# google/libultrahdr

Measured on AMD Instinct MI355X. Metric: Mpixels/s encode+decode (API-1 P010+YUV420, 4K), device-resident round trip, higher is better.
Workload: dtype f32; 1 GPU; API-1 3840x2160 round trip per step: encode (P010 HLG + YCbCr420 -> two-pass 3-ch gain map at scale 1, FDCT q95, Huffman: two JPEG scans) + decode (Huffman, IDCT, applyGainMap -> RGBA_F16 linear); frames resident in HBM

## Files before the change

### libultrahdr_amd/csrc/api_entropy.cpp

```cpp
#include "api_internal.h"

#include <condition_variable>
#include <functional>
#include <mutex>

uhdr_error_info_t uhdr_api::check_scan(const uhdr_hip_jpeg_scan_t* sc, bool need_coef, int* mcus_per_row, int* mcu_rows, int* blocks_per_mcu) {
  if (!sc) return err_status(UHDR_CODEC_INVALID_PARAM, "received nullptr for the scan description");
  if (sc->num_components != 1 && sc->num_components != 3)
    return err_status(UHDR_CODEC_INVALID_PARAM, "a scan has 1 or 3 components, received %d", sc->num_components);
  if (sc->w == 0 || sc->h == 0 || sc->w > 65535 || sc->h > 65535)
    return err_status(UHDR_CODEC_INVALID_PARAM, "image dimensions %ux%u are outside JPEG's 1..65535", sc->w, sc->h);
  int hmax = 1, vmax = 1, bpm = 0;
  for (int i = 0; i < sc->num_components; i++) {
    const int hs = sc->num_components == 1 ? 1 : sc->h_samp[i], vs = sc->num_components == 1 ? 1 : sc->v_samp[i];
    if (hs < 1 || hs > 2 || vs < 1 || vs > 2) return err_status(UHDR_CODEC_INVALID_PARAM, "component %d: sampling factors %dx%d not in {1, 2}", i, hs, vs);
    if (hs > hmax) hmax = hs;
    if (vs > vmax) vmax = vs;
    bpm += hs * vs;
    if (need_coef && (!sc->coef[i] || ((uintptr_t)sc->coef[i] & 15)))
      return err_status(UHDR_CODEC_INVALID_PARAM, "coefficient buffer %d is null or not 16-byte aligned", i);
    if (sc->blocks_w[i] < 1 || sc->blocks_h[i] < 1) return err_status(UHDR_CODEC_INVALID_PARAM, "component %d: empty block grid", i);
  }
  if (sc->num_components == 1) {
    *mcus_per_row = sc->blocks_w[0];
    *mcu_rows = sc->blocks_h[0];
    if ((unsigned)sc->blocks_w[0] != (sc->w + 7) / 8 || (unsigned)sc->blocks_h[0] != (sc->h + 7) / 8)
      return err_status(UHDR_CODEC_INVALID_PARAM, "a %dx%d block grid does not match a %ux%u image", sc->blocks_w[0], sc->blocks_h[0], sc->w, sc->h);
  } else {
    *mcus_per_row = (int)((sc->w + 8u * hmax - 1) / (8u * hmax));
    *mcu_rows = (int)((sc->h + 8u * vmax - 1) / (8u * vmax));
    for (int i = 0; i < 3; i++) {
      const unsigned cw = (sc->w * sc->h_samp[i] + hmax - 1) / hmax, chh = (sc->h * sc->v_samp[i] + vmax - 1) / vmax;
      const int min_w = (int)((cw + 7) / 8), min_h = (int)((chh + 7) / 8);
      if (sc->blocks_w[i] < min_w || sc->blocks_w[i] > *mcus_per_row * sc->h_samp[i] || sc->blocks_h[i] < min_h ||
          sc->blocks_h[i] > *mcu_rows * sc->v_samp[i])
        return err_status(UHDR_CODEC_INVALID_PARAM, "component %d: a %dx%d block grid does not match a %ux%u image at %dx%d sampling", i,
                          sc->blocks_w[i], sc->blocks_h[i], sc->w, sc->h, sc->h_samp[i], sc->v_samp[i]);
    }
  }
  *blocks_per_mcu = bpm;
  return ok_status();
}

static hipError_t wait_stream(uhdr_hip_ctx* c) {
  static const int spin_us = [] { const char* e = getenv("UHDR_HIP_SYNC_SPIN_US"); return e ? atoi(e) : 2000; }();
  if (spin_us > 0) {
    const auto t0 = std::chrono::steady_clock::now();
    for (;;) {
      const hipError_t q = hipStreamQuery(c->stream);
      if (q == hipSuccess) return hipSuccess;
      if (q != hipErrorNotReady) return q;
      if (std::chrono::steady_clock::now() - t0 > std::chrono::microseconds(spin_us)) break;
    }
  }
  return hipStreamSynchronize(c->stream);
}


uhdr_error_info_t uhdr_hip_huffman_encode_dev(uhdr_hip_ctx_t* c, const uhdr_hip_jpeg_scan_t* sc, uint8_t* out, size_t out_capacity,
                                              size_t* out_bytes) {
  if (!c) return err_status(UHDR_CODEC_INVALID_PARAM, "received nullptr for uhdr_hip context");
  if (!out || !out_bytes) return err_status(UHDR_CODEC_INVALID_PARAM, "received nullptr for the output buffer or size");
  int mpr = 0, mrows = 0, bpm = 0;
  UHDR_TRY(check_scan(sc, true, &mpr, &mrows, &bpm));
  const bool stream = sc->restart_interval == 0;
  if (!stream && (sc->restart_interval < 1 || sc->restart_interval > 65535 || sc->restart_interval * bpm > 64))
    return err_status(UHDR_CODEC_UNSUPPORTED_FEATURE, "restart_interval must be 0 (no markers) or in 1..%d for %d blocks per MCU (one wavefront "
                      "encodes one restart interval of at most 64 blocks); received %d", 64 / bpm, bpm, sc->restart_interval);
  if (stream && 2 * bpm > 64) return err_status(UHDR_CODEC_UNSUPPORTED_FEATURE, "%d blocks per MCU: outside the HIP path", bpm);
  HIP_TRY(hipSetDevice(c->device));
  if (!c->d_huff) {
    std::vector<uint32_t> blob(host::jpeg_huff_code_tables());
    blob.resize((size_t)host::kHuffTabWords + 16);
    memcpy(blob.data() + host::kHuffTabWords, host::jpeg_zigzag_to_natural(), 64);
    HIP_TRY(hipMalloc((void**)&c->d_huff, blob.size() * sizeof(uint32_t)));
    HIP_TRY(hipMemcpyAsync(c->d_huff, blob.data(), blob.size() * sizeof(uint32_t), hipMemcpyHostToDevice, c->stream));
    HIP_TRY(hipStreamSynchronize(c->stream));
  }
  HuffArgs a;
  memset(&a, 0, sizeof a);
  a.ncomp = sc->num_components;
  for (int i = 0; i < a.ncomp; i++) {
    a.coef[i] = sc->coef[i];
    a.bw[i] = sc->blocks_w[i]; a.bh[i] = sc->blocks_h[i];
    a.hs[i] = a.ncomp == 1 ? 1 : sc->h_samp[i]; a.vs[i] = a.ncomp == 1 ? 1 : sc->v_samp[i];
  }
  a.mcus_per_row = mpr;
  a.total_mcus = mpr * mrows;
  a.ri = stream ? huff_stream_segment_mcus(bpm) : sc->restart_interval;
  a.blocks_per_mcu = bpm;
  a.nseg = (a.total_mcus + a.ri - 1) / a.ri;
  a.tables = c->d_huff;
  a.zigzag = (const uint8_t*)(c->d_huff + host::kHuffTabWords);
  if (stream) {
    if (out_capacity > 0xFFFFFFF0u) out_capacity = 0xFFFFFFF0u;
    HuffStream t;
    memset(&t, 0, sizeof t);
    t.raw_words = ((uint64_t)out_capacity + 3) / 4 + 1;
    const uint64_t worst_words = (uint64_t)a.total_mcus * bpm * 52 + 2;
    if (t.raw_words > worst_words) t.raw_words = worst_words;
    const int nchunks = huff_stuff_chunks(t.raw_words * 4u);
    UHDR_TRY(ensure(c->scratch[4], (size_t)t.raw_words * 4));
    UHDR_TRY(ensure(c->scratch[5], ((size_t)a.nseg + 2) * sizeof(uint64_t) + (4 + (size_t)a.nseg + (size_t)nchunks) * sizeof(uint32_t)));
    t.raw = (uint32_t*)c->scratch[4].p;
    t.seg_start = (uint64_t*)c->scratch[5].p;
    uint64_t* d_total = t.seg_start + (size_t)a.nseg + 1;
    t.meta = (uint32_t*)(d_total + 1);
    t.seg_bits = t.meta + 4;
    uint32_t* chunk_counts = t.seg_bits + a.nseg;
    if (!c->huff_two_pass) {
      const size_t need = huff_stream_slot_bytes(a.nseg);
      if (c->huff_slots.cap >= need || !c->huff_slots_refused || need < c->huff_slots_refused) {
        if (ensure(c->huff_slots, need).error_code == UHDR_CODEC_OK) {
          t.slots = (uint32_t*)c->huff_slots.p;
        } else {
          (void)hipGetLastError();
          c->huff_slots_refused = need;
          fprintf(stderr, "uhdr_hip: no device memory for %zu bytes of Huffman segment slots: marker-less scans of that size take the two-pass route\n", need);
        }
      }
    }
    if (c->huff_route_log) fprintf(stderr, "uhdr_hip: huffman_encode stream route=%s nseg=%d\n", t.slots ? "one_walk" : "two_pass", a.nseg);
    {
      ProfScope ps(c, "huffman_encode");
      HIP_TRY(launch_huffman_encode_stream(a, t, chunk_counts, d_total, out, (uint64_t)out_capacity, c->stream));
    }
    c->stats.entropy_encode_stream++;
    if (!c->h_flags) HIP_TRY(hipHostMalloc((void**)&c->h_flags, 64 * sizeof(uint32_t), hipHostMallocDefault));
    uint32_t* hp = c->h_flags + 48;
    HIP_TRY(hipMemcpyAsync(hp, d_total, sizeof(uint64_t) + 4 * sizeof(uint32_t), hipMemcpyDeviceToHost, c->stream));
    HIP_TRY(wait_stream(c));
    uint64_t total = 0;
    uint32_t meta[4] = {0, 0, 0, 0};
    memcpy(&total, hp, sizeof total);
    memcpy(meta, hp + 2, sizeof meta);
    if (meta[2]) return err_status(UHDR_CODEC_INVALID_PARAM, "coefficients outside the baseline range (DC difference beyond 11 bits / AC beyond 10 bits)");
    const uint64_t raw_bytes = ((((uint64_t)meta[1] << 32) | meta[0]) + 7) / 8;
    if (raw_bytes > t.raw_words * 4u) total = raw_bytes + raw_bytes / 64 + 64;
    *out_bytes = (size_t)total;
    if (total > out_capacity)
      return err_status(UHDR_CODEC_MEM_ERROR, "entropy-coded data needs %llu bytes, the output buffer holds %zu", (unsigned long long)total, out_capacity);
    return ok_status();
  }
  a.slot_stride = huff_slot_stride();
  UHDR_TRY(ensure(c->scratch[4], (size_t)a.nseg * a.slot_stride));
  const size_t meta = (size_t)a.nseg * sizeof(uint32_t) + 16 + ((size_t)a.nseg + 1) * sizeof(uint64_t) + 16;
  UHDR_TRY(ensure(c->scratch[5], meta));
  a.slots = (uint8_t*)c->scratch[4].p;
  uint64_t* offsets = (uint64_t*)c->scratch[5].p;
  uint32_t* status = (uint32_t*)(offsets + (size_t)a.nseg + 1);
  a.seg_bytes = status + 2;
  {
    ProfScope ps(c, "huffman_encode");
    HIP_TRY(launch_huffman_encode(a, offsets, status, out, (uint64_t)out_capacity, c->stream));
  }
  c->stats.entropy_encode_intervals++;
  uint64_t total = 0;
  uint32_t bad = 0;
  HIP_TRY(hipMemcpyAsync(&total, offsets + a.nseg, sizeof total, hipMemcpyDeviceToHost, c->stream));
  HIP_TRY(hipMemcpyAsync(&bad, status, sizeof bad, hipMemcpyDeviceToHost, c->stream));
  HIP_TRY(wait_stream(c));
  if (bad) return err_status(UHDR_CODEC_INVALID_PARAM, "coefficients outside the baseline range (DC difference beyond 11 bits / AC beyond 10 bits)");
  *out_bytes = (size_t)total;
  if (total > out_capacity)
    return err_status(UHDR_CODEC_MEM_ERROR, "entropy-coded data needs %llu bytes, the output buffer holds %zu", (unsigned long long)total, out_capacity);
  return ok_status();
}

static bool make_dec_table(const uint8_t bits[17], const uint8_t vals[256], HuffDecTable* t) {
  memset(t, 0, sizeof *t);
  int nsym = 0;
  for (int l = 1; l <= 16; l++) nsym += bits[l];
  if (nsym > 256) return false;
  int code = 0, k = 0;
  for (int l = 1; l <= 16; l++) {
    if (bits[l]) {
// ... 744 lines not shown
```

### libultrahdr_amd/csrc/huffman_encode.hip

```cpp
#include "lds_copy.h"
#include "wg_scan.h"
#include "uhdr_types.h"

namespace uhdr {
namespace {

constexpr int kSegBlocks = 64;
constexpr int kWordsPerBlock = 52;
constexpr int kCoefRow = 33;

__device__ __forceinline__ uint32_t wave_incl_scan(uint32_t v, uint32_t lane) {
#pragma unroll
  for (int d = 1; d < 64; d <<= 1) {
    const uint32_t y = (uint32_t)__shfl_up((int)v, d, 64);
    if (lane >= (uint32_t)d) v += y;
  }
  return v;
}

__device__ __forceinline__ uint64_t zigzag_nonzero_map(const uint32_t* s_coef, uint32_t zz_of_lane, uint32_t lane) {
  uint64_t mine = 0;
  const uint32_t word = zz_of_lane >> 1, sh = (zz_of_lane & 1u) * 16u;
#pragma unroll 4
  for (uint32_t b = 0; b < (uint32_t)kSegBlocks; b++) {
    const uint32_t v = (s_coef[b * kCoefRow + word] >> sh) & 0xffffu;
    const uint64_t m = __builtin_amdgcn_ballot_w64(v != 0);
    if (lane == b) mine = m;
  }
  return mine;
}
template <typename Put>
__device__ __forceinline__ void walk_block(const uint32_t* dct, const uint32_t* act, int dc_diff, bool real, const uint32_t* coef_row,
                                           const uint8_t* zz, uint64_t nz, uint32_t& out_of_range, Put put) {
  int temp = dc_diff, temp2 = dc_diff;
  if (temp < 0) { temp = -temp; temp2--; }
  uint32_t nbits = 32u - (uint32_t)__clz(temp);
  out_of_range |= nbits > 11u;
  uint32_t e = dct[nbits & 15u];
  put(e & 0xffffu, e >> 16);
  if (nbits) put((uint32_t)temp2 & ((1u << nbits) - 1u), nbits);
  uint32_t prev = 0;
  if (real) {
    uint64_t m = nz & ~1ull;
    while (m != 0) {
      const uint32_t k = (uint32_t)__builtin_ctzll(m);
      m &= m - 1ull;
      uint32_t r = k - prev - 1u;
      prev = k;
      const uint32_t idx = zz[k];
      const uint32_t wd = coef_row[idx >> 1];
      temp = (idx & 1u) ? ((int)wd >> 16) : (int)(int16_t)(wd & 0xffffu);
      while (r > 15) {
        e = act[0xf0];
        put(e & 0xffffu, e >> 16);
        r -= 16;
      }
      temp2 = temp;
      if (temp < 0) { temp = -temp; temp2--; }
      nbits = 32u - (uint32_t)__clz(temp);
      out_of_range |= nbits > 10u;
      e = act[((r << 4) + nbits) & 255u];
      put(e & 0xffffu, e >> 16);
      put((uint32_t)temp2 & ((1u << (nbits & 31u)) - 1u), nbits);
    }
  }
  if (prev < 63u) {
    e = act[0];
    put(e & 0xffffu, e >> 16);
  }
}

constexpr int kWordsSmall = 16;
constexpr uint32_t kRetry = 0xFFFFFFFEu, kBadCoef = 0xFFFFFFFFu;

template <int WORDS, bool RETRY>
__global__ __launch_bounds__(64) void huff_encode_kernel(const HuffArgs a) {
  __shared__ __attribute__((aligned(16))) uint32_t s_tab[2 * (16 + 256)];
  __shared__ uint32_t s_coef[kSegBlocks * kCoefRow];
  __shared__ uint32_t s_bits[kSegBlocks * WORDS + 2];
  __shared__ int s_dc[kSegBlocks];
  __shared__ int s_real[kSegBlocks];
  __shared__ uint32_t s_gbits[kSegBlocks];
  __shared__ uint8_t s_zz[64];
  const uint32_t lane = threadIdx.x;
  copy_words_to_lds<4>(s_tab, a.tables, 2 * (16 + 256), lane, 64);
  s_zz[lane] = a.zigzag[lane];
  const int bpm = a.blocks_per_mcu;
  const int per = a.ri * bpm;
  const int G = (RETRY || per > 32) ? 1 : 64 / per;
  const uint32_t group_words = (uint32_t)(kSegBlocks * WORDS) / (uint32_t)G;
  const int nwseg = (a.nseg + G - 1) / G;

  for (int wseg = (int)blockIdx.x; wseg < nwseg; wseg += (int)gridDim.x) {
    __syncthreads();
    const int g = (int)lane / per, l = (int)lane - g * per;
    const int seg = wseg * G + g;
    if constexpr (RETRY) {
      if (a.seg_bytes[wseg] != kRetry) continue;
    }
    const int mcu_local = l / bpm, k_in_mcu = l - mcu_local * bpm;
    const int mcu = seg * a.ri + mcu_local;
    const bool active = g < G && seg < a.nseg && mcu_local < a.ri && mcu < a.total_mcus;
    int c = 0, kk = k_in_mcu;
    if (a.ncomp > 1) {
      while (c < a.ncomp - 1 && kk >= a.hs[c] * a.vs[c]) { kk -= a.hs[c] * a.vs[c]; c++; }
    }
    const int hs = a.ncomp > 1 ? a.hs[c] : 1, vs = a.ncomp > 1 ? a.vs[c] : 1;
    const int yi = kk / hs, xi = kk - yi * hs;
    const int my = mcu / a.mcus_per_row, mx = mcu - my * a.mcus_per_row;
    const int by = my * vs + yi, bx = mx * hs + xi;
    const bool real = active && by < a.bh[c] && bx < a.bw[c];
    uint32_t* crow = s_coef + lane * kCoefRow;
    if (real) {
      const uint4* src = (const uint4*)(a.coef[c] + ((size_t)by * a.bw[c] + bx) * 64);
#pragma unroll
      for (int i = 0; i < 8; i++) {
        const uint4 q = src[i];
        crow[4 * i] = q.x; crow[4 * i + 1] = q.y; crow[4 * i + 2] = q.z; crow[4 * i + 3] = q.w;
      }
    }
    s_real[lane] = real ? 1 : 0;
    s_dc[lane] = real ? (int)(int16_t)(crow[0] & 0xffffu) : 0;
    __syncthreads();
    int dcv = s_dc[lane];
    if (active && !real) {
      for (int d = 1; d <= 3; d++) {
        if (k_in_mcu >= d && s_real[lane - d]) { dcv = s_dc[lane - d]; break; }
      }
    }
    __syncthreads();
    s_dc[lane] = dcv;
    __syncthreads();
    int pred = 0;
    if (active) {
      if (kk > 0) pred = s_dc[lane - 1];
      else if (mcu_local > 0) pred = s_dc[(int)lane - bpm + hs * vs - 1];
    }
    const uint32_t* dct = s_tab + (c ? (16 + 256) : 0);
    const uint32_t* act = dct + 16;
    const int diff = dcv - pred;
    const uint64_t nz = zigzag_nonzero_map(s_coef, s_zz[lane], lane);

    uint32_t len = 0, oob = 0;
    if (active) walk_block(dct, act, diff, real, crow, s_zz, nz, oob, [&](uint32_t, uint32_t n) { len += n; });
    const uint32_t incl = wave_incl_scan(len, lane);
    const int first = g * per, last = min(first + per - 1, 63);
    const uint32_t v_before = (uint32_t)__shfl((int)incl, min(max(first - 1, 0), 63), 64);
    const uint32_t v_last = (uint32_t)__shfl((int)incl, last, 64);
    const uint32_t before = (first > 0 && first < 64) ? v_before : 0u;
    const uint32_t total_bits = g < G ? v_last - before : 0u;
    const uint32_t off = incl - len - before;
    const uint32_t cap_bits = group_words * 32u;
    if (__builtin_amdgcn_ballot_w64(oob != 0) != 0) {
      if (l == 0 && g < G && seg < a.nseg) a.seg_bytes[seg] = kBadCoef;
      continue;
    }
    const bool fits = total_bits <= cap_bits;
    if (l == 0 && g < G) s_gbits[g] = fits ? total_bits : 0xFFFFFFFFu;
    for (uint32_t i = lane; i < (uint32_t)(kSegBlocks * WORDS) + 2u; i += 64) s_bits[i] = 0u;
    __syncthreads();

    const uint32_t gbase = (uint32_t)g * group_words;
    if (active && fits) {
      uint64_t acc = 0;
      uint32_t cnt = off & 31u, w = gbase + (off >> 5);
      walk_block(dct, act, diff, real, crow, s_zz, nz, oob, [&](uint32_t code, uint32_t n) {
        acc = (acc << n) | (uint64_t)code;
        cnt += n;
        if (cnt >= 32u) {
          cnt -= 32u;
          atomicOr(&s_bits[w++], (uint32_t)(acc >> cnt));
        }
      });
      if (cnt) atomicOr(&s_bits[w], (uint32_t)(acc << (32u - cnt)));
    }
    __syncthreads();
    if (l == 0 && g < G && fits && (total_bits & 7u)) {
      const uint32_t pad = 8u - (total_bits & 7u), pos = total_bits & 31u;
      atomicOr(&s_bits[gbase + (total_bits >> 5)], ((1u << pad) - 1u) << (32u - pos - pad));
    }
    __syncthreads();

    for (int gg = 0; gg < G; gg++) {
      const int sg = wseg * G + gg;
      if (sg >= a.nseg) break;
      const uint32_t tb = s_gbits[gg];
      if (tb == 0xFFFFFFFFu) {
        if (lane == 0) a.seg_bytes[sg] = RETRY ? kBadCoef : kRetry;
        continue;
      }
      const uint32_t nbytes = (tb + 7u) >> 3;
      const uint32_t* bits = s_bits + (uint32_t)gg * group_words;
      uint8_t* dst = a.slots + (size_t)sg * a.slot_stride;
      uint32_t carry = 0;
      for (uint32_t base = 0; base < nbytes; base += 256) {
        const uint32_t i0 = base + lane * 4;
        const uint32_t wd = i0 < nbytes ? bits[i0 >> 2] : 0u;
        const uint32_t nv = i0 < nbytes ? min(nbytes - i0, 4u) : 0u;
        uint32_t b[4], nff = 0;
#pragma unroll
        for (int k = 0; k < 4; k++) {
          b[k] = (wd >> (24 - 8 * k)) & 0xffu;
          if ((uint32_t)k < nv && b[k] == 0xffu) nff++;
        }
        const uint32_t incl_ff = wave_incl_scan(nff, lane);
        uint32_t pos = i0 + carry + (incl_ff - nff);
#pragma unroll
        for (int k = 0; k < 4; k++) {
          if ((uint32_t)k < nv) {
            dst[pos++] = (uint8_t)b[k];
            if (b[k] == 0xffu) dst[pos++] = 0;
          }
        }
        carry += (uint32_t)__shfl((int)incl_ff, 63, 64);
      }
      if (lane == 0) a.seg_bytes[sg] = nbytes + carry;
    }
  }
}

__global__ __launch_bounds__(1024) void huff_offsets_kernel(const uint32_t* __restrict__ seg_bytes, int nseg, uint64_t* __restrict__ offsets,
                                                            uint32_t* __restrict__ status) {
  __shared__ uint64_t s_sum[1024];
  __shared__ uint32_t s_bad;
  const int tid = (int)threadIdx.x;
  if (tid == 0) s_bad = 0;
  __syncthreads();
  const int per = (nseg + 1023) / 1024, lo = min(tid * per, nseg), hi = min(lo + per, nseg);
  uint64_t sum = 0;
  bool bad = false;
  for (int i = lo; i < hi; i++) {
    const uint32_t n = seg_bytes[i];
    bad |= n >= kRetry;
    sum += (uint64_t)n + 2u;
  }
  if (bad) atomicOr(&s_bad, 1u);
  s_sum[tid] = sum;
  __syncthreads();
  for (int d = 1; d < 1024; d <<= 1) {
    const uint64_t y = tid >= d ? s_sum[tid - d] : 0;
    __syncthreads();
    s_sum[tid] += y;
    __syncthreads();
  }
  uint64_t run = s_sum[tid] - sum;
  for (int i = lo; i < hi; i++) {
    offsets[i] = run;
    run += (uint64_t)seg_bytes[i] + 2u;
  }
  if (tid == 1023) offsets[nseg] = s_sum[1023] - 2u;
  if (tid == 0) *status = s_bad;
}

__global__ __launch_bounds__(256) void huff_gather_kernel(const uint8_t* __restrict__ slots, uint32_t slot_stride,
                                                          const uint32_t* __restrict__ seg_bytes, const uint64_t* __restrict__ offsets, int nseg,
                                                          uint8_t* __restrict__ out, uint64_t cap) {
  for (int seg = (int)blockIdx.x; seg < nseg; seg += (int)gridDim.x) {
    const uint32_t n = seg_bytes[seg];
    const uint64_t off = offsets[seg];
    if (n >= kRetry || off + n + 2u > cap + (seg == nseg - 1 ? 2u : 0u)) continue;
    const uint8_t* src = slots + (size_t)seg * slot_stride;
    for (uint32_t i = threadIdx.x; i < n; i += 256) out[off + i] = src[i];
    if (threadIdx.x == 0 && seg < nseg - 1) {
      out[off + n] = 0xff;
      out[off + n + 1] = (uint8_t)(0xd0 + (seg & 7));
    }
  }
}


constexpr int kStuffChunk = 4096;

template <int WORDS, int PASS>
__global__ __launch_bounds__(64) void huff_stream_kernel(const HuffArgs a, const HuffStream t) {
  __shared__ __attribute__((aligned(16))) uint32_t s_tab[2 * (16 + 256)];
  __shared__ uint32_t s_coef[kSegBlocks * kCoefRow];
  __shared__ uint32_t s_bits[PASS == 0 ? 1 : kSegBlocks * WORDS + 2];
  __shared__ int s_dc[kSegBlocks];
  __shared__ int s_real[kSegBlocks];
  __shared__ uint8_t s_zz[64];
  const uint32_t lane = threadIdx.x;
  if constexpr (PASS == 2) {
    if (t.meta[3] == 0) return;
  }
  copy_words_to_lds<4>(s_tab, a.tables, 2 * (16 + 256), lane, 64);
  s_zz[lane] = a.zigzag[lane];
  const int bpm = a.blocks_per_mcu;
  constexpr uint32_t kCapBits = (uint32_t)(kSegBlocks * WORDS) * 32u;
  for (int seg = (int)blockIdx.x; seg < a.nseg; seg += (int)gridDim.x) {
    __syncthreads();
    uint64_t start = 0;
    uint32_t seg_total = 0;
    if constexpr (PASS != 0) {
      seg_total = t.seg_bits[seg];
      start = t.seg_start[seg];
      const bool small = seg_total + 32u <= (uint32_t)(kSegBlocks * kWordsSmall) * 32u;
      if (seg_total >= kRetry || small != (PASS == 1)) continue;
    }
    const int mcu_local = (int)lane / bpm, k_in_mcu = (int)lane - mcu_local * bpm;
    const int mcu = seg * a.ri + mcu_local - 1;
    const bool valid = mcu_local <= a.ri && mcu >= 0 && mcu < a.total_mcus;
    const bool emits = valid && mcu_local >= 1;
    int c = 0, kk = k_in_mcu;
    if (a.ncomp > 1) {
      while (c < a.ncomp - 1 && kk >= a.hs[c] * a.vs[c]) { kk -= a.hs[c] * a.vs[c]; c++; }
    }
    const int hs = a.ncomp > 1 ? a.hs[c] : 1, vs = a.ncomp > 1 ? a.vs[c] : 1;
    const int yi = kk / hs, xi = kk - yi * hs;
    const int mcu_c = valid ? mcu : 0;
    const int my = mcu_c / a.mcus_per_row, mx = mcu_c - my * a.mcus_per_row;
    const int by = my * vs + yi, bx = mx * hs + xi;
    const bool real = valid && by < a.bh[c] && bx < a.bw[c];
    uint32_t* crow = s_coef + lane * kCoefRow;
    if (real) {
      const uint4* src = (const uint4*)(a.coef[c] + ((size_t)by * a.bw[c] + bx) * 64);
      if (emits) {
#pragma unroll
        for (int i = 0; i < 8; i++) {
          const uint4 q = src[i];
          crow[4 * i] = q.x; crow[4 * i + 1] = q.y; crow[4 * i + 2] = q.z; crow[4 * i + 3] = q.w;
        }
      } else {
        crow[0] = *(const uint32_t*)src;
      }
    }
    s_real[lane] = real ? 1 : 0;
    s_dc[lane] = real ? (int)(int16_t)(crow[0] & 0xffffu) : 0;
    __syncthreads();
    int dcv = s_dc[lane];
    if (valid && !real) {
      for (int d = 1; d <= 3; d++) {
        if (k_in_mcu >= d && s_real[lane - d]) { dcv = s_dc[lane - d]; break; }
      }
    }
    __syncthreads();
    s_dc[lane] = dcv;
    __syncthreads();
    int pred = 0;
    if (emits) {
      if (kk > 0) pred = s_dc[lane - 1];
      else pred = s_dc[(int)lane - bpm + hs * vs - 1];
    }
    const uint32_t* dct = s_tab + (c ? (16 + 256) : 0);
    const uint32_t* act = dct + 16;
    const int diff = dcv - pred;
    const uint64_t nz = zigzag_nonzero_map(s_coef, s_zz[lane], lane);
    uint32_t len = 0, oob = 0;
    if (emits) walk_block(dct, act, diff, real, crow, s_zz, nz, oob, [&](uint32_t, uint32_t n) { len += n; });
    const uint32_t incl = wave_incl_scan(len, lane);
    const uint32_t total_bits = (uint32_t)__shfl((int)incl, 63, 64);
    if constexpr (PASS == 0) {
      const bool bad = __builtin_amdgcn_ballot_w64(oob != 0) != 0;
      if (lane == 0) t.seg_bits[seg] = bad ? kBadCoef : total_bits;
    } else {
      const uint32_t phase = (uint32_t)(start & 31u);
      if (phase + total_bits > kCapBits) continue;
      const uint32_t nwords = (phase + total_bits + 31u) >> 5;
      for (uint32_t i = lane; i < nwords + 1u; i += 64) s_bits[i] = 0u;
      __syncthreads();
      if (emits) {
        const uint32_t off = phase + incl - len;
        uint64_t acc = 0;
        uint32_t cnt = off & 31u, w = off >> 5;
        walk_block(dct, act, diff, real, crow, s_zz, nz, oob, [&](uint32_t code, uint32_t n) {
          acc = (acc << n) | (uint64_t)code;
          cnt += n;
          if (cnt >= 32u) {
            cnt -= 32u;
            atomicOr(&s_bits[w++], (uint32_t)(acc >> cnt));
          }
        });
        if (cnt) atomicOr(&s_bits[w], (uint32_t)(acc << (32u - cnt)));
      }
      __syncthreads();
      const uint64_t end_bit = start + total_bits;
      if (seg == a.nseg - 1 && lane == 0 && (end_bit & 7u)) {
        const uint32_t e = phase + total_bits, pad = 8u - (e & 7u), pos = e & 31u;
        s_bits[e >> 5] |= ((1u << pad) - 1u) << (32u - pos - pad);
      }
      __syncthreads();
      const uint64_t w0 = start >> 5;
      const uint32_t tail = (phase + total_bits) & 31u;
      for (uint32_t i = lane; i < nwords; i += 64) {
        if (w0 + i >= t.raw_words) break;
        const uint32_t v = __builtin_bswap32(s_bits[i]);
        const bool shared = (i == 0 && phase != 0) || (i == nwords - 1 && tail != 0);
        if (shared) atomicOr(&t.raw[w0 + i], v);
        else t.raw[w0 + i] = v;
      }
    }
  }
}

constexpr int kWalkSegs = 4;
constexpr int kSlotWords = kSegBlocks * kWordsSmall;
__device__ __forceinline__ void wave_sync() {
  __builtin_amdgcn_fence(__ATOMIC_SEQ_CST, "wavefront");
  __builtin_amdgcn_wave_barrier();
}
__global__ __launch_bounds__(64 * kWalkSegs) void huff_stream_walk_kernel(const HuffArgs a, const HuffStream t) {
  __shared__ __attribute__((aligned(16))) uint32_t s_tab[2 * (16 + 256)];
  __shared__ uint32_t s_coef_all[kWalkSegs][kSegBlocks * kCoefRow];
  __shared__ uint32_t s_bits_all[kWalkSegs][kSlotWords];
  __shared__ uint8_t s_zz[64];
  const uint32_t lane = threadIdx.x & 63u, wv = threadIdx.x >> 6;
  copy_words_to_lds<4>(s_tab, a.tables, 2 * (16 + 256), threadIdx.x, 64 * kWalkSegs);
  if (threadIdx.x < 64) s_zz[threadIdx.x] = a.zigzag[threadIdx.x];
  __syncthreads();
  uint32_t* s_coef = s_coef_all[wv];
  uint32_t* s_bits = s_bits_all[wv];
  const int bpm = a.blocks_per_mcu;
  const int mcu_local = (int)lane / bpm, k_in_mcu = (int)lane - mcu_local * bpm;
  int c = 0, kk = k_in_mcu;
  if (a.ncomp > 1) {
    while (c < a.ncomp - 1 && kk >= a.hs[c] * a.vs[c]) { kk -= a.hs[c] * a.vs[c]; c++; }
  }
  const int hs = a.ncomp > 1 ? a.hs[c] : 1, vs = a.ncomp > 1 ? a.vs[c] : 1;
  const int yi = kk / hs, xi = kk - yi * hs;
  const int pred_lane = (kk > 0 ? (int)lane - 1 : (int)lane - bpm + hs * vs - 1) & 63;
  const uint32_t* dct = s_tab + (c ? (16 + 256) : 0);
  const uint32_t* act = dct + 16;
  const uint32_t zz_of_lane = s_zz[lane];
  uint32_t* crow = s_coef + lane * kCoefRow;
  for (int seg = (int)blockIdx.x * kWalkSegs + (int)wv; seg < a.nseg; seg += (int)gridDim.x * kWalkSegs) {
    wave_sync();
    const int mcu = seg * a.ri + mcu_local - 1;
    const bool valid = mcu_local <= a.ri && mcu >= 0 && mcu < a.total_mcus;
    const bool emits = valid && mcu_local >= 1;
    const int mcu_c = valid ? mcu : 0;
    const int my = mcu_c / a.mcus_per_row, mx = mcu_c - my * a.mcus_per_row;
    const int by = my * vs + yi, bx = mx * hs + xi;
    const bool real = valid && by < a.bh[c] && bx < a.bw[c];
    int dc0 = 0;
    if (real) {
      const uint4* src = (const uint4*)(a.coef[c] + ((size_t)by * a.bw[c] + bx) * 64);
      if (emits) {
        uint4 q[8];
#pragma unroll
        for (int i = 0; i < 8; i++) q[i] = src[i];
#pragma unroll
        for (int i = 0; i < 8; i++) { crow[4 * i] = q[i].x; crow[4 * i + 1] = q[i].y; crow[4 * i + 2] = q[i].z; crow[4 * i + 3] = q[i].w; }
        dc0 = (int)(int16_t)(q[0].x & 0xffffu);
      } else {
        dc0 = (int)(int16_t)(*(const uint32_t*)src & 0xffffu);
      }
    }
    const uint64_t real_mask = __builtin_amdgcn_ballot_w64(real);
    const int up1 = __shfl_up(dc0, 1, 64), up2 = __shfl_up(dc0, 2, 64), up3 = __shfl_up(dc0, 3, 64);
    int dcv = dc0;
    if (valid && !real) {
      if (k_in_mcu >= 1 && ((real_mask >> (lane - 1)) & 1ull)) dcv = up1;
      else if (k_in_mcu >= 2 && ((real_mask >> (lane - 2)) & 1ull)) dcv = up2;
      else if (k_in_mcu >= 3 && ((real_mask >> (lane - 3)) & 1ull)) dcv = up3;
    }
    const int pred_v = __shfl(dcv, pred_lane, 64);
    const int diff = dcv - (emits ? pred_v : 0);
    wave_sync();
    const uint64_t nz = zigzag_nonzero_map(s_coef, zz_of_lane, lane);
    uint32_t len = 0, oob = 0;
    if (emits) walk_block(dct, act, diff, real, crow, s_zz, nz, oob, [&](uint32_t, uint32_t n) { len += n; });
    const uint32_t incl = wave_incl_scan(len, lane);
    const uint32_t total_bits = (uint32_t)__shfl((int)incl, 63, 64);
    const bool bad = __builtin_amdgcn_ballot_w64(oob != 0) != 0;
    if (lane == 0) t.seg_bits[seg] = bad ? kBadCoef : total_bits;
    if (bad || total_bits + 32u > (uint32_t)kSlotWords * 32u) continue;
    const uint32_t nwords = (total_bits + 31u) >> 5;
    for (uint32_t i = lane; i < nwords + 1u; i += 64) s_bits[i] = 0u;
    wave_sync();
    if (emits) {
      const uint32_t off = incl - len;
      uint64_t acc = 0;
      uint32_t cnt = off & 31u, w = off >> 5;
      walk_block(dct, act, diff, real, crow, s_zz, nz, oob, [&](uint32_t code, uint32_t n) {
        acc = (acc << n) | (uint64_t)code;
        cnt += n;
        if (cnt >= 32u) {
          cnt -= 32u;
          atomicOr(&s_bits[w++], (uint32_t)(acc >> cnt));
        }
      });
      if (cnt) atomicOr(&s_bits[w], (uint32_t)(acc << (32u - cnt)));
    }
    wave_sync();
    uint32_t* slot = t.slots + (size_t)seg * (size_t)kSlotWords;
    for (uint32_t i = lane; i < nwords; i += 64) slot[i] = s_bits[i];
  }
}

constexpr int kPlaceSegs = 4;
__global__ __launch_bounds__(64 * kPlaceSegs) void huff_stream_place_kernel(int nseg, const HuffStream t) {
  const uint32_t lane = threadIdx.x & 63u;
  const int seg = (int)blockIdx.x * kPlaceSegs + (int)(threadIdx.x >> 6);
  if (seg >= nseg) return;
  const uint32_t total_bits = t.seg_bits[seg];
  if (total_bits >= kRetry || total_bits + 32u > (uint32_t)(kSegBlocks * kWordsSmall) * 32u) return;
  const uint64_t start = t.seg_start[seg];
  const uint32_t phase = (uint32_t)(start & 31u);
  const uint32_t nin = (total_bits + 31u) >> 5, nwords = (phase + total_bits + 31u) >> 5;
  const uint32_t e = phase + total_bits, tail = e & 31u;
  const bool flush = seg == nseg - 1 && (e & 7u);
  const uint32_t* slot = t.slots + (size_t)seg * (size_t)(kSegBlocks * kWordsSmall);
  const uint64_t w0 = start >> 5;
  for (uint32_t i = lane; i < nwords; i += 64) {
    if (w0 + i >= t.raw_words) break;
    const uint32_t cur = i < nin ? slot[i] : 0u, prev = (i > 0 && phase != 0) ? slot[i - 1] : 0u;
    uint32_t v = __builtin_amdgcn_alignbit(prev, cur, phase);
    if (flush && i == (e >> 5)) {
      const uint32_t pad = 8u - (e & 7u);
      v |= ((1u << pad) - 1u) << (32u - tail - pad);
    }
    v = __builtin_bswap32(v);
    const bool shared = (i == 0 && phase != 0) || (i == nwords - 1 && tail != 0);
    if (shared) atomicOr(&t.raw[w0 + i], v);
    else t.raw[w0 + i] = v;
  }
}

template <int NT = 1024, typename Sink>
__device__ __forceinline__ uint64_t wg_scan_tiles(const uint32_t* __restrict__ v, int n, uint32_t* s_val , uint64_t* s_sum , Sink sink) {
  const int tid = (int)threadIdx.x;
  uint64_t carry = 0;
  for (int base = 0; base < n; base += 8 * NT) {
    uint32_t ld[8];
#pragma unroll
    for (int j = 0; j < 8; j++) ld[j] = v[min(base + j * NT + tid, n - 1)];
#pragma unroll
    for (int j = 0; j < 8; j++) s_val[j * NT + tid] = base + j * NT + tid < n ? ld[j] : 0u;
    __syncthreads();
    uint32_t x[8];
    uint64_t sum = 0;
#pragma unroll
    for (int j = 0; j < 8; j++) { x[j] = s_val[tid * 8 + j]; sum += x[j]; }
    uint64_t sc[1] = {sum}, all[1];
    wg_incl_scan<NT, 1>(sc, s_sum, all);
    uint64_t run = carry + sc[0] - sum;
#pragma unroll
    for (int j = 0; j < 8; j++) {
      const int i = base + tid * 8 + j;
      if (i < n) sink(i, x[j], run);
      run += x[j];
    }
    carry += all[0];
  }
  return carry;
}

constexpr int kStreamScanThreads = 256;
__global__ __launch_bounds__(kStreamScanThreads) void huff_stream_scan_kernel(const uint32_t* __restrict__ seg_bits, int nseg, const HuffStream t) {
  __shared__ uint32_t s_val[8 * kStreamScanThreads];
  __shared__ uint64_t s_sum[kStreamScanThreads / 64];
  __shared__ uint32_t s_bad;
  const int tid = (int)threadIdx.x;
  if (tid == 0) s_bad = 0;
  __syncthreads();
  bool bad = false;
  uint32_t big = 0;
  const uint64_t total = wg_scan_tiles<kStreamScanThreads>(seg_bits, nseg, s_val, s_sum, [&](int i, uint32_t n, uint64_t run) {
    bad |= n >= kRetry;
    big += (n < kRetry && n + 32u > (uint32_t)(kSegBlocks * kWordsSmall) * 32u) ? 1u : 0u;
    t.seg_start[i] = run;
    if ((run >> 5) < t.raw_words) t.raw[run >> 5] = 0u;
  });
  if (bad) atomicOr(&s_bad, 1u);
  if (big) atomicAdd(&s_bad, big << 1);
  __syncthreads();
  if (tid == kStreamScanThreads - 1) {
    t.seg_start[nseg] = total;
    if ((total >> 5) < t.raw_words) t.raw[total >> 5] = 0u;
// ... 136 lines not shown
```

### libultrahdr_amd/csrc/lds_copy.h

```cpp
#ifndef UHDR_LDS_COPY_H
#define UHDR_LDS_COPY_H
#include <hip/hip_runtime.h>
#include <stdint.h>

namespace uhdr {

template <int UNROLL = 8>
__device__ __forceinline__ void copy_words_to_lds(uint32_t* dst, const uint32_t* __restrict__ src, uint32_t nwords, uint32_t tid, uint32_t nthreads) {
  const uint4* s4 = (const uint4*)src;
  uint4* d4 = (uint4*)dst;
  const uint32_t nv = nwords >> 2;
  for (uint32_t i = tid; i < nv; i += UNROLL * nthreads) {
    uint4 v[UNROLL];
#pragma unroll
    for (int u = 0; u < UNROLL; u++) {
      const uint32_t j = i + (uint32_t)u * nthreads;
      v[u] = s4[j < nv ? j : i];
    }
#pragma unroll
    for (int u = 0; u < UNROLL; u++) {
      const uint32_t j = i + (uint32_t)u * nthreads;
      d4[j < nv ? j : i] = v[u];
    }
  }
}

template <int UNROLL = 8>
__device__ __forceinline__ void copy_to_lds(void* dst_, const void* __restrict__ src_, uint32_t nwords, uint32_t tid, uint32_t nthreads) {
  uint32_t* dst = (uint32_t*)dst_;
  const uint32_t* src = (const uint32_t*)src_;
  if ((((uintptr_t)src | (uintptr_t)dst) & 15u) == 0) {
    const uint32_t body = nwords & ~3u;
    copy_words_to_lds<UNROLL>(dst, src, body, tid, nthreads);
    if (body + tid < nwords) dst[body + tid] = src[body + tid];
    return;
  }
  for (uint32_t i = tid; i < nwords; i += UNROLL * nthreads) {
    uint32_t v[UNROLL];
#pragma unroll
    for (int u = 0; u < UNROLL; u++) {
      const uint32_t j = i + (uint32_t)u * nthreads;
      v[u] = src[j < nwords ? j : i];
    }
#pragma unroll
    for (int u = 0; u < UNROLL; u++) {
      const uint32_t j = i + (uint32_t)u * nthreads;
      dst[j < nwords ? j : i] = v[u];
    }
  }
}

}
#endif
```

### libultrahdr_amd/csrc/uhdr_types.h

```cpp
#pragma once
#include <hip/hip_runtime.h>
#include <stdint.h>

#include "device_math.h"
#include "uhdr_hip.h"

namespace uhdr {

struct ImageView {
  const void* p[3];
  uint32_t stride[3];
  uint32_t w, h;
  int fmt;
  int range;
};
struct ImageViewMut {
  void* p[3];
  uint32_t stride[3];
  uint32_t w, h;
  int fmt;
  int range;
};

constexpr int kSrgbN = 1024;
// ... 166 lines not shown
  Rgb2Yuv base_k;
  ImageViewMut ycc;
};

struct YuvXformParams {
  ImageViewMut img;
  Mat3 c;
};
struct RgbToYcbcrParams {
  ImageView src;
  ImageViewMut dst;
  Rgb2Yuv k;
};

hipError_t launch_apply_gainmap(const ApplyParams& p, hipStream_t s);
hipError_t launch_apply_gainmap_coef(const ApplyParams& p, hipStream_t s);
int apply_quad_mode(const ApplyParams& p);
hipError_t launch_generate_gainmap(const GenParams& p, bool two_pass, hipStream_t s);
hipError_t launch_generate_gainmap_coef(const GenParams& p, const CoefSrc& cs, int vsamp, bool two_pass, hipStream_t s);
int gen_coef_partials_count(const GenParams& p);
hipError_t launch_affine_map(const AffineParams& p, hipStream_t s);
hipError_t launch_minmax_table(const MinmaxTableParams& p, hipStream_t s);
hipError_t launch_map_blocks(const float* ratio, const AffineDev* dev, const double* math_tab, int nch, int bw, int bh, const uint16_t* qt_luma,
                             const uint16_t* qt_chroma, int16_t* const coef[3], uint8_t* map_out, uint32_t out_stride, hipStream_t s);
hipError_t launch_map_blocks_onepass(const GenParams& g, int nch, const uint16_t* qt_luma, const uint16_t* qt_chroma, int16_t* const coef[3],
                                     uint8_t* map_out, uint32_t out_stride, hipStream_t s);
hipError_t launch_base_blocks(const ImageView& yuv420, const Mat3* c, const uint16_t* qt_luma, const uint16_t* qt_chroma, int16_t* const coef[3],
                              hipStream_t s);
hipError_t launch_base_blocks_rgba(const ImageView& rgba, const Rgb2Yuv& k, const Mat3* c, const uint16_t* qt_luma, const uint16_t* qt_chroma,
                                   int16_t* const coef[3], hipStream_t s);
hipError_t launch_selftest(int which, unsigned long long* out, uint32_t arg0, uint32_t arg1, uint32_t seed, const double* math_tab, const AffineDev* dev,
                           hipStream_t s);
int gen_partials_count(const GenParams& p);
hipError_t launch_encode_api0_fused(const FusedParams& p, bool two_pass, int* grid_out, hipStream_t s);
bool encode_api0_p010_layout_ok(const ImageView& hdr, const ImageView& base420);
hipError_t launch_encode_api0_p010_fused(const FusedParams& p, bool two_pass, int* grid_out, hipStream_t s);
bool encode_api0_fused_scaled_layout_ok(const FusedParams& p);
hipError_t launch_encode_api0_fused_scaled(const FusedParams& p, hipStream_t s);
hipError_t launch_encode_api0_p010_fused_scaled(const FusedParams& p, hipStream_t s);
hipError_t launch_tone_map(const ToneMapParams& p, hipStream_t s);
hipError_t launch_transform_yuv(const YuvXformParams& p, hipStream_t s);
hipError_t launch_rgb_to_ycbcr(const RgbToYcbcrParams& p, hipStream_t s);
struct FdctEdge {
  int on, w, h, col_mode, fill, mcu_rows;
};
hipError_t launch_fdct_quant(const uint8_t* plane, size_t stride, int bw, int bh,
                             const uint16_t* qt_host, int16_t* coef, hipStream_t s, const FdctEdge* edge = nullptr);

hipError_t launch_fdct_quant_rgb(const uint8_t* rgb, size_t pitch, int bpp, int bw, int bh, const uint16_t* qt_luma_host,
                                 const uint16_t* qt_chroma_host, int16_t* coef_y, int16_t* coef_cb, int16_t* coef_cr, hipStream_t s, int vw = 0,
                                 int vh = 0);
hipError_t launch_repack(int mode, const void* src, size_t src_pitch, void* dst, size_t dst_pitch, uint32_t w, uint32_t h,
                         hipStream_t s);
struct EffectPlane {
  const void* src;
  void* dst;
  uint32_t elem;
  uint32_t src_w, src_h, src_stride;
  uint32_t dst_w, dst_h, dst_stride;
  uint32_t mode;
  uint32_t a0, a1;
};
hipError_t launch_effect_plane(const EffectPlane& p, hipStream_t s);
struct ResizePlane {
  const void* src;
  void* dst;
  uint32_t src_w, src_h, dst_w;
  uint32_t rows, y0;
  size_t src_pitch, dst_pitch;
  double scale_x, scale_y;
};
hipError_t launch_resize_image(const ResizePlane& p, int bpp, hipStream_t s);

struct HuffArgs {
  const int16_t* coef[3];
  int bw[3], bh[3];
  int hs[3], vs[3];
  int ncomp;
  int mcus_per_row, total_mcus;
  int ri;
  int blocks_per_mcu;
  int nseg;
  const uint32_t* tables;
  const uint8_t* zigzag;
  uint8_t* slots;
  uint32_t slot_stride;
  uint32_t* seg_bytes;
};
uint32_t huff_slot_stride();
struct HuffStream {
  uint32_t* seg_bits;
  uint64_t* seg_start;
  uint32_t* raw;
  uint64_t raw_words;
  uint32_t* meta;
  uint32_t* slots;
};
int huff_stream_segment_mcus(int blocks_per_mcu);
size_t huff_stream_slot_bytes(int nseg);
int huff_stuff_chunks(uint64_t raw_bytes);
hipError_t launch_huffman_encode_stream(const HuffArgs& a, const HuffStream& t, uint32_t* chunk_counts, uint64_t* out_bytes, uint8_t* out, uint64_t cap,
                                        hipStream_t s);
hipError_t launch_huffman_encode(const HuffArgs& a, uint64_t* offsets, uint32_t* status, uint8_t* out, uint64_t cap, hipStream_t s);

struct HuffDecTable {
  uint16_t lut[512];
  int maxcode[18];
  int valoff[17];
  uint8_t vals[256];
};
struct HuffDecArgs {
  const uint8_t* data;
  uint32_t nbytes;
  const uint32_t* starts;
  const uint32_t* ends;
  int nseg, ri, total_mcus, mcus_per_row, ncomp;
  int bw[3], bh[3], hs[3], vs[3];
  int16_t* coef[3];
  const HuffDecTable* tabs;
  const uint8_t* zigzag;
  uint32_t* status;
};
constexpr int kHuffL2Max = 16;
struct HuffFastTable {
  uint16_t l1[512];
  uint16_t l2[kHuffL2Max][128];
};
constexpr int kHuffValWords = 512 + kHuffL2Max * 128;
constexpr int kHuffPairBits = 10, kHuffPairWords = 1 << kHuffPairBits;
constexpr int kHuffL2Total = 32;
constexpr int kHuffPairBlobWords = 4 * kHuffPairWords + kHuffL2Total * 128 / 2;
constexpr int kHuffPairValBlobWords = 8 * kHuffPairWords + kHuffL2Total * 128 / 2;
struct HuffSyncArgs {
  const uint8_t* clean;
  uint32_t nbytes;
  const uint32_t* nstuffed;
  uint32_t sub_bits;
  uint64_t* state[2];
  uint8_t* changed[2];
  uint32_t* nblk;
  uint32_t* scan_tmp;
  uint32_t* flags;
  int* dcd;
  uint32_t total_blocks;
  int blocks_per_mcu, ncomp, mcus_per_row;
  int bw[3], bh[3], hs[3], vs[3], first_blk[3];
  uint8_t comp_of[16];
  int16_t* coef[3];
  const HuffFastTable* ftabs;
  const HuffFastTable* ttabs;
  const uint32_t* vtabs;
  const uint32_t* ptabs;
  const uint32_t* pvtabs;
  const uint8_t* zigzag;
  int hyp_h, hyp_levels;
  uint64_t* hyp_state;
  uint8_t* hyp_map;
  uint16_t* hyp_cnt;
  int hyp_hist;
  int hyp_main_levels;
  int strag_levels;
  uint32_t* strag_list;
  uint32_t strag_cap;
  int16_t* coef_scan;
  int write_form;
  uint32_t total_mcus;
  uint4* zero_ptr[3];
// ... 47 lines not shown
```

Measured before the change: 12720 Mpixels/s.

## Stage Huffman coefficients in zigzag order and software-pipeline the AC walk

Coefficients are now permuted into zigzag order while being staged into LDS, using a compile-time table. This removes the per-coefficient zigzag indirection and the LDS zigzag table, so the nonzero ballot map reads one contiguous uint16 column. The AC walk is restructured to prefetch the next two coefficients and their table entries ahead of use, fuses each code with its magnitude bits into a single put, and hoists the out-of-range check out of the loop. The stream walk kernel's slot write-back now uses 16-byte vector copies. The cost is more register pressure from the unrolled permutation and the prefetch state, and the vector write-back may store up to three padding words past nwords.

```diff
diff --git a/libultrahdr_amd/csrc/api_entropy.cpp b/libultrahdr_amd/csrc/api_entropy.cpp
--- a/libultrahdr_amd/csrc/api_entropy.cpp
+++ b/libultrahdr_amd/csrc/api_entropy.cpp
@@ -91,7 +91,6 @@
   a.blocks_per_mcu = bpm;
   a.nseg = (a.total_mcus + a.ri - 1) / a.ri;
   a.tables = c->d_huff;
-  a.zigzag = (const uint8_t*)(c->d_huff + host::kHuffTabWords);
   if (stream) {
     if (out_capacity > 0xFFFFFFF0u) out_capacity = 0xFFFFFFF0u;
     HuffStream t;
diff --git a/libultrahdr_amd/csrc/huff_zigzag.h b/libultrahdr_amd/csrc/huff_zigzag.h
--- /dev/null
+++ b/libultrahdr_amd/csrc/huff_zigzag.h
@@ -0,0 +1,12 @@
+#ifndef UHDR_HUFF_ZIGZAG_H
+#define UHDR_HUFF_ZIGZAG_H
+#include <stdint.h>
+
+namespace uhdr {
+
+constexpr uint8_t kHuffZigzag[64] = {0,  1,  8,  16, 9,  2,  3,  10, 17, 24, 32, 25, 18, 11, 4,  5,  12, 19, 26, 33, 40, 48,
+                                     41, 34, 27, 20, 13, 6,  7,  14, 21, 28, 35, 42, 49, 56, 57, 50, 43, 36, 29, 22, 15, 23,
+                                     30, 37, 44, 51, 58, 59, 52, 45, 38, 31, 39, 46, 53, 60, 61, 54, 47, 55, 62, 63};
+
+}
+#endif
diff --git a/libultrahdr_amd/csrc/huffman_encode.hip b/libultrahdr_amd/csrc/huffman_encode.hip
--- a/libultrahdr_amd/csrc/huffman_encode.hip
+++ b/libultrahdr_amd/csrc/huffman_encode.hip
@@ -1,3 +1,4 @@
+#include "huff_zigzag.h"
 #include "lds_copy.h"
 #include "wg_scan.h"
 #include "uhdr_types.h"
@@ -18,12 +19,30 @@
   return v;
 }
 
-__device__ __forceinline__ uint64_t zigzag_nonzero_map(const uint32_t* s_coef, uint32_t zz_of_lane, uint32_t lane) {
+__device__ __forceinline__ int stage_row_zigzag(uint32_t* crow, const uint4* __restrict__ src) {
+  uint4 q[8];
+#pragma unroll
+  for (int i = 0; i < 8; i++) q[i] = src[i];
+  const auto word = [&](int n) -> uint32_t {
+    const uint4& v = q[n >> 2];
+    return (n & 3) == 0 ? v.x : (n & 3) == 1 ? v.y : (n & 3) == 2 ? v.z : v.w;
+  };
+#pragma unroll
+  for (int j = 0; j < 32; j++) {
+    const int lo = kHuffZigzag[2 * j], hi = kHuffZigzag[2 * j + 1];
+    const uint32_t l16 = (lo & 1) ? word(lo >> 1) >> 16 : word(lo >> 1) & 0xffffu;
+    const uint32_t h16 = (hi & 1) ? word(hi >> 1) & 0xffff0000u : word(hi >> 1) << 16;
+    crow[j] = l16 | h16;
+  }
+  return (int)(int16_t)(q[0].x & 0xffffu);
+}
+
+__device__ __forceinline__ uint64_t zigzag_nonzero_map(const uint32_t* s_coef, uint32_t lane) {
   uint64_t mine = 0;
-  const uint32_t word = zz_of_lane >> 1, sh = (zz_of_lane & 1u) * 16u;
-#pragma unroll 4
+  const uint16_t* col = (const uint16_t*)s_coef + lane;
+#pragma unroll 8
   for (uint32_t b = 0; b < (uint32_t)kSegBlocks; b++) {
-    const uint32_t v = (s_coef[b * kCoefRow + word] >> sh) & 0xffffu;
+    const uint32_t v = col[b * (2 * kCoefRow)];
     const uint64_t m = __builtin_amdgcn_ballot_w64(v != 0);
     if (lane == b) mine = m;
   }
@@ -31,43 +50,67 @@
 }
 template <typename Put>
 __device__ __forceinline__ void walk_block(const uint32_t* dct, const uint32_t* act, int dc_diff, bool real, const uint32_t* coef_row,
-                                           const uint8_t* zz, uint64_t nz, uint32_t& out_of_range, Put put) {
+                                           uint64_t nz, uint32_t& out_of_range, Put put) {
+  const uint16_t* row = (const uint16_t*)coef_row;
   int temp = dc_diff, temp2 = dc_diff;
   if (temp < 0) { temp = -temp; temp2--; }
-  uint32_t nbits = 32u - (uint32_t)__clz(temp);
+  const uint32_t nbits = 32u - (uint32_t)__clz(temp);
   out_of_range |= nbits > 11u;
-  uint32_t e = dct[nbits & 15u];
-  put(e & 0xffffu, e >> 16);
-  if (nbits) put((uint32_t)temp2 & ((1u << nbits) - 1u), nbits);
-  uint32_t prev = 0;
-  if (real) {
-    uint64_t m = nz & ~1ull;
-    while (m != 0) {
-      const uint32_t k = (uint32_t)__builtin_ctzll(m);
-      m &= m - 1ull;
-      uint32_t r = k - prev - 1u;
-      prev = k;
-      const uint32_t idx = zz[k];
-      const uint32_t wd = coef_row[idx >> 1];
-      temp = (idx & 1u) ? ((int)wd >> 16) : (int)(int16_t)(wd & 0xffffu);
-      while (r > 15) {
-        e = act[0xf0];
-        put(e & 0xffffu, e >> 16);
-        r -= 16;
-      }
-      temp2 = temp;
-      if (temp < 0) { temp = -temp; temp2--; }
-      nbits = 32u - (uint32_t)__clz(temp);
-      out_of_range |= nbits > 10u;
-      e = act[((r << 4) + nbits) & 255u];
-      put(e & 0xffffu, e >> 16);
-      put((uint32_t)temp2 & ((1u << (nbits & 31u)) - 1u), nbits);
-    }
-  }
-  if (prev < 63u) {
-    e = act[0];
-    put(e & 0xffffu, e >> 16);
-  }
+  const uint32_t e = dct[nbits & 15u], e_eob = act[0];
+  uint64_t m = real ? nz & ~1ull : 0ull;
+  const bool eob = (m >> 63) == 0;
+  uint32_t left = (uint32_t)__builtin_popcountll(m);
+  const auto next_pos = [&]() -> uint32_t {
+    const uint32_t k = (uint32_t)__builtin_ctzll(m | (1ull << 63));
+    m &= m - 1ull;
+    return k;
+  };
+  const auto size_of = [](uint16_t raw, uint32_t& bits) -> uint32_t {
+    int t = (int)(int16_t)raw, t2 = t;
+    if (t < 0) { t = -t; t2--; }
+    const uint32_t nb = 32u - (uint32_t)__clz(t);
+    bits = (uint32_t)t2 & ((1u << (nb & 31u)) - 1u);
+    return nb;
+  };
+  uint32_t kA = 0, kB = 0, kC = 0, nbA = 0, bitsA = 0, rA = 0, e_zrl = 0, max_nb = 0;
+  uint16_t v0 = 0, v1 = 0;
+  uint32_t e0 = 0, e1 = 0;
+  if (left) {
+    kA = next_pos();
+    const uint16_t vA = row[kA];
+    kB = next_pos();
+    v0 = row[kB];
+    kC = next_pos();
+    e_zrl = act[0xf0];
+    rA = kA - 1u;
+    nbA = size_of(vA, bitsA);
+    e0 = act[((rA << 4) + nbA) & 255u];
+  }
+  put(((e & 0xffffu) << (nbits & 31u)) | ((uint32_t)temp2 & ((1u << (nbits & 31u)) - 1u)), (e >> 16) + nbits);
+  const auto step = [&](uint16_t v_next, uint16_t& v_after, uint32_t e_cur, uint32_t& e_next) {
+    v_after = row[kC];
+    uint32_t bitsB;
+    const uint32_t rB = kB - kA - 1u, nbB = size_of(v_next, bitsB);
+    e_next = act[((rB << 4) + nbB) & 255u];
+    uint32_t r = rA;
+    while (r > 15) {
+      put(e_zrl & 0xffffu, e_zrl >> 16);
+      r -= 16;
+    }
+    max_nb = max(max_nb, nbA);
+    put(((e_cur & 0xffffu) << nbA) | bitsA, (e_cur >> 16) + nbA);
+    kA = kB; rA = rB; nbA = nbB; bitsA = bitsB;
+    kB = kC;
+    kC = next_pos();
+  };
+  while (left != 0) {
+    step(v0, v1, e0, e1);
+    if (--left == 0) break;
+    step(v1, v0, e1, e0);
+    --left;
+  }
+  out_of_range |= max_nb > 10u;
+  if (eob) put(e_eob & 0xffffu, e_eob >> 16);
 }
 
 constexpr int kWordsSmall = 16;
@@ -81,10 +124,8 @@
   __shared__ int s_dc[kSegBlocks];
   __shared__ int s_real[kSegBlocks];
   __shared__ uint32_t s_gbits[kSegBlocks];
-  __shared__ uint8_t s_zz[64];
   const uint32_t lane = threadIdx.x;
   copy_words_to_lds<4>(s_tab, a.tables, 2 * (16 + 256), lane, 64);
-  s_zz[lane] = a.zigzag[lane];
   const int bpm = a.blocks_per_mcu;
   const int per = a.ri * bpm;
   const int G = (RETRY || per > 32) ? 1 : 64 / per;
@@ -111,16 +152,10 @@
     const int by = my * vs + yi, bx = mx * hs + xi;
     const bool real = active && by < a.bh[c] && bx < a.bw[c];
     uint32_t* crow = s_coef + lane * kCoefRow;
-    if (real) {
-      const uint4* src = (const uint4*)(a.coef[c] + ((size_t)by * a.bw[c] + bx) * 64);
-#pragma unroll
-      for (int i = 0; i < 8; i++) {
-        const uint4 q = src[i];
-        crow[4 * i] = q.x; crow[4 * i + 1] = q.y; crow[4 * i + 2] = q.z; crow[4 * i + 3] = q.w;
-      }
-    }
+    int dc0 = 0;
+    if (real) dc0 = stage_row_zigzag(crow, (const uint4*)(a.coef[c] + ((size_t)by * a.bw[c] + bx) * 64));
     s_real[lane] = real ? 1 : 0;
-    s_dc[lane] = real ? (int)(int16_t)(crow[0] & 0xffffu) : 0;
+    s_dc[lane] = dc0;
     __syncthreads();
     int dcv = s_dc[lane];
     if (active && !real) {
@@ -139,10 +174,10 @@
     const uint32_t* dct = s_tab + (c ? (16 + 256) : 0);
     const uint32_t* act = dct + 16;
     const int diff = dcv - pred;
-    const uint64_t nz = zigzag_nonzero_map(s_coef, s_zz[lane], lane);
+    const uint64_t nz = zigzag_nonzero_map(s_coef, lane);
 
     uint32_t len = 0, oob = 0;
-    if (active) walk_block(dct, act, diff, real, crow, s_zz, nz, oob, [&](uint32_t, uint32_t n) { len += n; });
+    if (active) walk_block(dct, act, diff, real, crow, nz, oob, [&](uint32_t, uint32_t n) { len += n; });
     const uint32_t incl = wave_incl_scan(len, lane);
     const int first = g * per, last = min(first + per - 1, 63);
     const uint32_t v_before = (uint32_t)__shfl((int)incl, min(max(first - 1, 0), 63), 64);
@@ -164,7 +199,7 @@
     if (active && fits) {
       uint64_t acc = 0;
       uint32_t cnt = off & 31u, w = gbase + (off >> 5);
-      walk_block(dct, act, diff, real, crow, s_zz, nz, oob, [&](uint32_t code, uint32_t n) {
+      walk_block(dct, act, diff, real, crow, nz, oob, [&](uint32_t code, uint32_t n) {
         acc = (acc << n) | (uint64_t)code;
         cnt += n;
         if (cnt >= 32u) {
@@ -278,13 +313,11 @@
   __shared__ uint32_t s_bits[PASS == 0 ? 1 : kSegBlocks * WORDS + 2];
   __shared__ int s_dc[kSegBlocks];
   __shared__ int s_real[kSegBlocks];
-  __shared__ uint8_t s_zz[64];
   const uint32_t lane = threadIdx.x;
   if constexpr (PASS == 2) {
     if (t.meta[3] == 0) return;
   }
   copy_words_to_lds<4>(s_tab, a.tables, 2 * (16 + 256), lane, 64);
-  s_zz[lane] = a.zigzag[lane];
   const int bpm = a.blocks_per_mcu;
   constexpr uint32_t kCapBits = (uint32_t)(kSegBlocks * WORDS) * 32u;
   for (int seg = (int)blockIdx.x; seg < a.nseg; seg += (int)gridDim.x) {
@@ -312,20 +345,14 @@
     const int by = my * vs + yi, bx = mx * hs + xi;
     const bool real = valid && by < a.bh[c] && bx < a.bw[c];
     uint32_t* crow = s_coef + lane * kCoefRow;
+    int dc0 = 0;
     if (real) {
       const uint4* src = (const uint4*)(a.coef[c] + ((size_t)by * a.bw[c] + bx) * 64);
-      if (emits) {
-#pragma unroll
-        for (int i = 0; i < 8; i++) {
-          const uint4 q = src[i];
-          crow[4 * i] = q.x; crow[4 * i + 1] = q.y; crow[4 * i + 2] = q.z; crow[4 * i + 3] = q.w;
-        }
-      } else {
-        crow[0] = *(const uint32_t*)src;
-      }
+      if (emits) dc0 = stage_row_zigzag(crow, src);
+      else dc0 = (int)(int16_t)(*(const uint32_t*)src & 0xffffu);
     }
     s_real[lane] = real ? 1 : 0;
-    s_dc[lane] = real ? (int)(int16_t)(crow[0] & 0xffffu) : 0;
+    s_dc[lane] = dc0;
     __syncthreads();
     int dcv = s_dc[lane];
     if (valid && !real) {
@@ -344,9 +371,9 @@
     const uint32_t* dct = s_tab + (c ? (16 + 256) : 0);
     const uint32_t* act = dct + 16;
     const int diff = dcv - pred;
-    const uint64_t nz = zigzag_nonzero_map(s_coef, s_zz[lane], lane);
+    const uint64_t nz = zigzag_nonzero_map(s_coef, lane);
     uint32_t len = 0, oob = 0;
-    if (emits) walk_block(dct, act, diff, real, crow, s_zz, nz, oob, [&](uint32_t, uint32_t n) { len += n; });
+    if (emits) walk_block(dct, act, diff, real, crow, nz, oob, [&](uint32_t, uint32_t n) { len += n; });
     const uint32_t incl = wave_incl_scan(len, lane);
     const uint32_t total_bits = (uint32_t)__shfl((int)incl, 63, 64);
     if constexpr (PASS == 0) {
@@ -362,7 +389,7 @@
         const uint32_t off = phase + incl - len;
         uint64_t acc = 0;
         uint32_t cnt = off & 31u, w = off >> 5;
-        walk_block(dct, act, diff, real, crow, s_zz, nz, oob, [&](uint32_t code, uint32_t n) {
+        walk_block(dct, act, diff, real, crow, nz, oob, [&](uint32_t code, uint32_t n) {
           acc = (acc << n) | (uint64_t)code;
           cnt += n;
           if (cnt >= 32u) {
@@ -401,11 +428,9 @@
 __global__ __launch_bounds__(64 * kWalkSegs) void huff_stream_walk_kernel(const HuffArgs a, const HuffStream t) {
   __shared__ __attribute__((aligned(16))) uint32_t s_tab[2 * (16 + 256)];
   __shared__ uint32_t s_coef_all[kWalkSegs][kSegBlocks * kCoefRow];
-  __shared__ uint32_t s_bits_all[kWalkSegs][kSlotWords];
-  __shared__ uint8_t s_zz[64];
+  __shared__ __attribute__((aligned(16))) uint32_t s_bits_all[kWalkSegs][kSlotWords];
   const uint32_t lane = threadIdx.x & 63u, wv = threadIdx.x >> 6;
   copy_words_to_lds<4>(s_tab, a.tables, 2 * (16 + 256), threadIdx.x, 64 * kWalkSegs);
-  if (threadIdx.x < 64) s_zz[threadIdx.x] = a.zigzag[threadIdx.x];
   __syncthreads();
   uint32_t* s_coef = s_coef_all[wv];
   uint32_t* s_bits = s_bits_all[wv];
@@ -420,7 +445,6 @@
   const int pred_lane = (kk > 0 ? (int)lane - 1 : (int)lane - bpm + hs * vs - 1) & 63;
   const uint32_t* dct = s_tab + (c ? (16 + 256) : 0);
   const uint32_t* act = dct + 16;
-  const uint32_t zz_of_lane = s_zz[lane];
   uint32_t* crow = s_coef + lane * kCoefRow;
   for (int seg = (int)blockIdx.x * kWalkSegs + (int)wv; seg < a.nseg; seg += (int)gridDim.x * kWalkSegs) {
     wave_sync();
@@ -435,12 +459,7 @@
     if (real) {
       const uint4* src = (const uint4*)(a.coef[c] + ((size_t)by * a.bw[c] + bx) * 64);
       if (emits) {
-        uint4 q[8];
-#pragma unroll
-        for (int i = 0; i < 8; i++) q[i] = src[i];
-#pragma unroll
-        for (int i = 0; i < 8; i++) { crow[4 * i] = q[i].x; crow[4 * i + 1] = q[i].y; crow[4 * i + 2] = q[i].z; crow[4 * i + 3] = q[i].w; }
-        dc0 = (int)(int16_t)(q[0].x & 0xffffu);
+        dc0 = stage_row_zigzag(crow, src);
       } else {
         dc0 = (int)(int16_t)(*(const uint32_t*)src & 0xffffu);
       }
@@ -456,9 +475,9 @@
     const int pred_v = __shfl(dcv, pred_lane, 64);
     const int diff = dcv - (emits ? pred_v : 0);
     wave_sync();
-    const uint64_t nz = zigzag_nonzero_map(s_coef, zz_of_lane, lane);
+    const uint64_t nz = zigzag_nonzero_map(s_coef, lane);
     uint32_t len = 0, oob = 0;
-    if (emits) walk_block(dct, act, diff, real, crow, s_zz, nz, oob, [&](uint32_t, uint32_t n) { len += n; });
+    if (emits) walk_block(dct, act, diff, real, crow, nz, oob, [&](uint32_t, uint32_t n) { len += n; });
     const uint32_t incl = wave_incl_scan(len, lane);
     const uint32_t total_bits = (uint32_t)__shfl((int)incl, 63, 64);
     const bool bad = __builtin_amdgcn_ballot_w64(oob != 0) != 0;
@@ -471,7 +490,7 @@
       const uint32_t off = incl - len;
       uint64_t acc = 0;
       uint32_t cnt = off & 31u, w = off >> 5;
-      walk_block(dct, act, diff, real, crow, s_zz, nz, oob, [&](uint32_t code, uint32_t n) {
+      walk_block(dct, act, diff, real, crow, nz, oob, [&](uint32_t code, uint32_t n) {
         acc = (acc << n) | (uint64_t)code;
         cnt += n;
         if (cnt >= 32u) {
@@ -483,7 +502,7 @@
     }
     wave_sync();
     uint32_t* slot = t.slots + (size_t)seg * (size_t)kSlotWords;
-    for (uint32_t i = lane; i < nwords; i += 64) slot[i] = s_bits[i];
+    copy_words_from_lds<4>(slot, s_bits, nwords, lane, 64);
   }
 }
 
diff --git a/libultrahdr_amd/csrc/lds_copy.h b/libultrahdr_amd/csrc/lds_copy.h
--- a/libultrahdr_amd/csrc/lds_copy.h
+++ b/libultrahdr_amd/csrc/lds_copy.h
@@ -5,11 +5,8 @@
 
 namespace uhdr {
 
-template <int UNROLL = 8>
-__device__ __forceinline__ void copy_words_to_lds(uint32_t* dst, const uint32_t* __restrict__ src, uint32_t nwords, uint32_t tid, uint32_t nthreads) {
-  const uint4* s4 = (const uint4*)src;
-  uint4* d4 = (uint4*)dst;
-  const uint32_t nv = nwords >> 2;
+template <int UNROLL>
+__device__ __forceinline__ void copy_vec16(uint4* d4, const uint4* __restrict__ s4, uint32_t nv, uint32_t tid, uint32_t nthreads) {
   for (uint32_t i = tid; i < nv; i += UNROLL * nthreads) {
     uint4 v[UNROLL];
 #pragma unroll
@@ -23,6 +20,16 @@
       d4[j < nv ? j : i] = v[u];
     }
   }
+}
+
+template <int UNROLL = 8>
+__device__ __forceinline__ void copy_words_to_lds(uint32_t* dst, const uint32_t* __restrict__ src, uint32_t nwords, uint32_t tid, uint32_t nthreads) {
+  copy_vec16<UNROLL>((uint4*)dst, (const uint4*)src, nwords >> 2, tid, nthreads);
+}
+
+template <int UNROLL = 4>
+__device__ __forceinline__ void copy_words_from_lds(uint32_t* __restrict__ dst, const uint32_t* src, uint32_t nwords, uint32_t tid, uint32_t nthreads) {
+  copy_vec16<UNROLL>((uint4*)dst, (const uint4*)src, (nwords + 3u) >> 2, tid, nthreads);
 }
 
 template <int UNROLL = 8>
diff --git a/libultrahdr_amd/csrc/uhdr_types.h b/libultrahdr_amd/csrc/uhdr_types.h
--- a/libultrahdr_amd/csrc/uhdr_types.h
+++ b/libultrahdr_amd/csrc/uhdr_types.h
@@ -272,7 +272,6 @@
   int blocks_per_mcu;
   int nseg;
   const uint32_t* tables;
-  const uint8_t* zigzag;
   uint8_t* slots;
   uint32_t slot_stride;
   uint32_t* seg_bytes;
```

Measured after the change: 13100 Mpixels/s (median of 6 runs). +3.0%, better.
